# huangnengCSU/NanoSNP

Hardware: AMD Instinct MI355X
Metric: candidate SNP sites/sec (pileup encode + model fwd), 30x windows (higher is better)
Workload: dtype f32; 1 GPU; BASELINE configs[1]: pileup encode + PileupModel fwd, 1M synthetic 30x windows (G2) resident in HBM, batch=4096; batch=4096, windows_resident_per_gpu=1048576, streams=32, precision=fp32, parallelism=site-sharded x1, rooted gather of calls, world_size_observed=1, gather=torch

## Files before the change

nanosnp_amd/csrc/pileup_encode.hip:

```cpp
#include "nsnp_common.hpp"
#include <math.h>

namespace {

enum { CH_A = 0, CH_C, CH_G, CH_T, CH_I, CH_I1, CH_D, CH_D1, CH_STAR,
       CH_a, CH_c, CH_g, CH_t, CH_i, CH_i1, CH_d, CH_d1, CH_POUND, NCH };

constexpr int ENC_BLOCK = 256;
constexpr int MAX_INDEL = 60;

__device__ __forceinline__ int byte_class(int b)
{
    switch (b) {
    case 'A': return 0; case 'C': return 1; case 'G': return 2; case 'T': return 3;
    case 'a': return 4; case 'c': return 5; case 'g': return 6; case 't': return 7;
    case '*': return 8; case '#': return 9;
    case '+': return 11; case '-': return 12; case '^': return 13;
    default: return 10;
    }
}
__device__ __forceinline__ bool is_fwd_char(int b)
{
    return b == 'A' || b == 'C' || b == 'G' || b == 'T' || b == 'N' || b == '*';
}
// ... 73 lines not shown
    Quad t{0, 0, 0, 0};
    for (int64_t i = begin; i < end;) {
        const int b = bases[i];
        const int cls = byte_class(b);
        if (cls < 10) {
            c.k0 += cls == 0; c.k1 += cls == 1; c.k2 += cls == 2; c.k3 += cls == 3; c.k4 += cls == 4;
            c.k5 += cls == 5; c.k6 += cls == 6; c.k7 += cls == 7; c.k8 += cls == 8; c.k9 += cls == 9;
            ++i;
        } else if (cls == 11 || cls == 12) {
            ++i;
            long long adv = 0;
            while (i < end && bases[i] >= '0' && bases[i] <= '9') { adv = adv > 100000000 ? adv : adv * 10 + (bases[i] - '0'); ++i; }
            if (adv <= MAX_INDEL) {
                const int64_t avail = end - i;
                const int len = (int)(adv < avail ? adv : avail);
                t.inc((b == '-' ? 2 : 0) + (len > 0 && is_fwd_char(bases[i]) ? 0 : 1));
            }
            i = adv < end - i ? i + adv : end;
        } else if (cls == 13) i += 2;
        else ++i;
    }
    cnt = c; tot = t;
    mx = rescan_maxima(bases, begin, end);
}

template <typename P>
__device__ __forceinline__ int max_del_exact(P bases, int64_t begin, int64_t end)
{
    int md = 0;
    for (int64_t i = begin; i < end;) {
        const int b = bases[i];
        if (b == '+' || b == '-') {
            ++i;
            long long adv = 0;
            while (i < end && bases[i] >= '0' && bases[i] <= '9') { adv = adv > 100000000 ? adv : adv * 10 + (bases[i] - '0'); ++i; }
            if (b == '-' && adv <= MAX_INDEL && adv > md) md = (int)adv;
            i = adv < end - i ? i + adv : end;
        } else if (b == '^') i += 2;
        else ++i;
    }
    return md;
}

__device__ __forceinline__ bool bed_bit(const uint32_t* __restrict__ bits, int64_t n_bits, int64_t i)
{
    return i >= 0 && i < n_bits && ((bits[i >> 5] >> (i & 31)) & 1u);
}
__device__ __forceinline__ bool bed_any(const uint32_t* __restrict__ bits, int64_t n_bits, int64_t lo, int64_t hi)
{
    if (lo < 0) lo = 0;
    if (hi > n_bits) hi = n_bits;
    if (lo >= hi) return false;
    const int64_t w0 = lo >> 5, w1 = (hi - 1) >> 5;
    for (int64_t w = w0; w <= w1; ++w) {
        uint32_t m = 0xffffffffu;
        if (w == w0) m &= 0xffffffffu << (lo & 31);
        if (w == w1) m &= 0xffffffffu >> (31 - ((hi - 1) & 31));
        if (bits[w] & m) return true;
    }
    return false;
}

constexpr int KEY_SHIFT = 36;
struct BedTable { const uint32_t* words; const int64_t* bed_off; const int64_t* seq_off; int64_t n_contigs; };

__device__ __forceinline__ const uint32_t* bed_table_contig(const BedTable& t, int64_t key, int64_t& n_bits)
{
    const int64_t cid = key >> KEY_SHIFT;
    n_bits = 0;
    if (cid < 0 || cid >= t.n_contigs) return nullptr;
    const int64_t w0 = t.bed_off[cid], cap = (t.bed_off[cid + 1] - w0) * 32, len = t.seq_off[cid + 1] - t.seq_off[cid];
    n_bits = len < cap ? len : cap;
    return t.words + w0;
}
__device__ __forceinline__ int64_t key_pos(int64_t key) { return key & ((1ll << KEY_SHIFT) - 1); }

struct AfThreshold { uint64_t t; int k; int mode; };

static AfThreshold make_af_threshold(double a)
{
    AfThreshold r{0, 0, 0};
    if (a != a) { r.mode = 2; return r; }
    if (a <= 0.0) { r.mode = 1; return r; }
    int e = 0;
    const double m = frexp(a, &e);
    if (!(m > 0.0) || e > 40) { r.mode = 2; return r; }
    const uint64_t M53 = (uint64_t)ldexp(m, 53);
    const bool pow2 = M53 == (1ull << 52);
    r.t = pow2 ? 4 * M53 - 1 : 2 * M53 - 1;
    r.k = (pow2 ? 55 : 54) - e;
    if (r.k >= 88) { r.mode = 1; r.t = 0; r.k = 0; }
    if (r.k < 0) { r.mode = 2; }
    return r;
}

struct AfTable { uint32_t w[128]; };

static AfTable make_af_table(const AfThreshold& af)
{
    AfTable t;
    uint16_t m[256];
    for (int d = 0; d < 256; ++d) {
        m[d] = 0xffff;
        if (af.mode == 1) { m[d] = 1; continue; }
        if (af.mode == 2) continue;
        const unsigned __int128 rhs = (unsigned __int128)af.t * (uint32_t)(d ? d : 1);
        int lo = 1, hi = (d ? d : 1) + 1;
        while (lo < hi) {
            const int c = (lo + hi) >> 1;
            if ((((unsigned __int128)(uint32_t)c) << af.k) >= rhs) hi = c; else lo = c + 1;
        }
        if (lo <= (d ? d : 1)) m[d] = (uint16_t)lo;
    }
    for (int i = 0; i < 128; ++i) t.w[i] = (uint32_t)m[2 * i] | ((uint32_t)m[2 * i + 1] << 16);
    return t;
}

constexpr int ENC_WAVES = ENC_BLOCK / 64;
#ifndef NSNP_ENC_STAGE
#define NSNP_ENC_STAGE 5120
#endif
#ifndef NSNP_ENC_ECAP
#define NSNP_ENC_ECAP 208
#endif
constexpr int STAGE_BYTES = NSNP_ENC_STAGE;
constexpr int ENC_ECAP = NSNP_ENC_ECAP;
#ifndef NSNP_ENC_P3STEP
#define NSNP_ENC_P3STEP 4
#endif
constexpr int P3_STEP = NSNP_ENC_P3STEP;
constexpr int ENC_NBLK = 8;
static_assert(STAGE_BYTES >= 64 * NCH * 4, "the stage buffer doubles as the 64 x 18 output transposition buffer");
static_assert(STAGE_BYTES <= 8192, "staged positions are kept in 13 bits");
static_assert(4 * (ENC_WAVES * (STAGE_BYTES + (ENC_ECAP + P3_STEP) * 8 + 64 * 32) + 4096 + 2 * 512) <= 160 * 1024, "four blocks per CU (LDS)");
constexpr int ENC_ECAP_BED = ENC_ECAP - 32;
static_assert(4 * (ENC_WAVES * (STAGE_BYTES + (ENC_ECAP_BED + P3_STEP) * 8 + 64 * 36) + 4096 + 2 * 512) <= 160 * 1024, "four blocks per CU (LDS)");

struct EncBed { const int64_t* pos; const uint32_t* bits; int64_t n_bits; int32_t* max_del; };
struct EncKeys { const int64_t* key; BedTable tab; int32_t* max_del; };
enum { ENC_PLAIN = 0, ENC_BED = 1, ENC_KEYS = 2 };

__device__ __forceinline__ int wave_scan_incl(int v)
{
    int x = v;
    x += __builtin_amdgcn_update_dpp(0, x, 0x111, 0xf, 0xf, true);
    x += __builtin_amdgcn_update_dpp(0, x, 0x112, 0xf, 0xf, true);
    x += __builtin_amdgcn_update_dpp(0, x, 0x114, 0xf, 0xf, true);
    x += __builtin_amdgcn_update_dpp(0, x, 0x118, 0xf, 0xf, true);
    x += __builtin_amdgcn_update_dpp(0, x, 0x142, 0xa, 0xf, true);
    x += __builtin_amdgcn_update_dpp(0, x, 0x143, 0xc, 0xf, true);
    return x;
}

#ifndef NSNP_ENC_MINW
#define NSNP_ENC_MINW 4
#endif
template <int MODE, typename Bed>
__device__ __forceinline__ void encode_columns_body(
    const uint8_t* __restrict__ bases, const int64_t* __restrict__ col_off, const uint8_t* __restrict__ ref,
    int64_t M, const AfThreshold& af, const AfTable& aft, const AfThreshold& afi, const AfTable& afti, int min_cov, int32_t* __restrict__ counts,
    int32_t* __restrict__ depth_out,
    uint8_t* __restrict__ flags, const Bed& bed)
{
    constexpr bool BED = MODE != ENC_PLAIN;
    constexpr int ECAP = BED ? ENC_ECAP_BED : ENC_ECAP;
    constexpr int NACC = BED ? 9 : 8;
    __shared__ uint32_t af_min[128];
    __shared__ uint32_t afi_min[128];
    __shared__ __attribute__((aligned(16))) uint8_t stage_b[ENC_WAVES][STAGE_BYTES];
    __shared__ uint2 ents[ENC_WAVES][ECAP + P3_STEP];
    __shared__ uint32_t colacc[ENC_WAVES][NACC][64];
    __shared__ uint4 tab[256];
    const int tid = threadIdx.x, lane = tid & 63, wave = tid >> 6;
    {
        const int cls = byte_class(tid);
        uint4 r{0u, 0u, 0u, 0u};
        if (cls < 4) r.x = 1u << (8 * cls);
        else if (cls < 8) r.y = 1u << (8 * (cls - 4));
        else if (cls < 10) r.z = 1u << (8 * (cls - 8));
        else if (cls >= 11) r.w = 1u;
        if (is_fwd_char(tid)) r.z |= 1u << 24;
        tab[tid ^ ((tid >> 2) & 12)] = r;
        if (tid < 128) { af_min[tid] = aft.w[tid]; afi_min[tid] = afti.w[tid]; }
        if (tid < ENC_WAVES * P3_STEP) ents[tid / P3_STEP][tid % P3_STEP] = uint2{0x80000000u, 0u};
    }
    __syncthreads();
    const int64_t wave_col0 = ((int64_t)blockIdx.x * ENC_WAVES + wave) * 64;
    if (wave_col0 >= M) return;
    const int64_t c = wave_col0 + lane;
    const bool live = c < M;
    const int n_live = (int)(M - wave_col0 < 64 ? M - wave_col0 : 64);
    const int64_t* __restrict__ woff = col_off + wave_col0;
    const int64_t wave_end = woff[n_live];
    const int64_t begin64 = woff[lane < n_live ? lane : n_live];
    const int refraw = (ref + wave_col0)[lane < n_live ? lane : n_live - 1];
    const int64_t total = col_off[M];
    const int64_t wave_b0 = __builtin_amdgcn_readfirstlane((int)(begin64 & 0xffffffff)) |
                            ((int64_t)__builtin_amdgcn_readfirstlane((int)(begin64 >> 32)) << 32);
    constexpr int REL_SAT = 1 << 30;
    const int64_t rb64 = begin64 - wave_b0;
    int rbeg = (int)(rb64 < REL_SAT ? rb64 : REL_SAT);
    int rend = __shfl_down(rbeg, 1);
    {
        const int64_t re64 = wave_end - wave_b0;
        if (lane == n_live - 1) rend = (int)(re64 < REL_SAT ? re64 : REL_SAT);
    }
    if (!live) { rbeg = 0; rend = 0; }
    const uint8_t* __restrict__ wbase = bases + wave_b0;

    uint8_t* st = stage_b[wave];
    const uint32_t* st32 = reinterpret_cast<const uint32_t*>(st);
    uint2* ent = ents[wave] + P3_STEP;
    uint32_t (*const cacc)[64] = colacc[wave];
    int32_t cnt[10];
#pragma unroll
    for (int k = 0; k < 10; ++k) cnt[k] = 0;
    Quad tot{0, 0, 0, 0};
    Quad mx{0, 0, 0, 0};
    bool slow = false;
    int mdel = 0;

    for (int first = 0; first < n_live;) {
        const int b0 = __builtin_amdgcn_readlane(rbeg, first);
        const int mis = (int)((uintptr_t)(wbase + b0) & 15);
        const uint8_t* __restrict__ src = wbase + (b0 - mis);
        const bool fits = live && lane >= first && b0 < REL_SAT && rend <= (STAGE_BYTES - 16 - mis) + b0 && rend >= b0;
        const unsigned long long fm = __ballot(fits) >> first;
        int n_fit = (~fm) ? __builtin_ctzll(~fm) : 64;
        if (n_fit > n_live - first) n_fit = n_live - first;
        if (n_fit == 0) {
            if (lane == first) slow = true;
            first += 1;
            continue;
        }
        const int last = first + n_fit;
        const int span = __builtin_amdgcn_readlane(rend, last - 1) - b0 + mis;
        {
            const bool inside = (uintptr_t)src >= (uintptr_t)bases && (uintptr_t)src + (((uintptr_t)span + 15) & ~(uintptr_t)15) <= (uintptr_t)(bases + total);
            if (inside) {
                constexpr int NP = (STAGE_BYTES + 1023) / 1024;
                const int o_last = ((span - 1) >> 4) << 4;
                uint4 pc[NP];
#pragma unroll
                for (int i = 0; i < NP; ++i) { const int o = (lane + 64 * i) * 16; pc[i] = *reinterpret_cast<const uint4*>(src + (o < span ? o : o_last)); }
#pragma unroll
                for (int i = 0; i < NP; ++i) { const int o = (lane + 64 * i) * 16; if (o < span) *reinterpret_cast<uint4*>(st + o) = pc[i]; }
            } else {
                for (int o = lane * 16; o < span; o += 64 * 16) {
                    uint32_t wv[4] = {0u, 0u, 0u, 0u};
                    for (int k = 0; k < 16; ++k) {
                        const uint8_t* q = src + o + k;
                        if (q >= bases && q < bases + total) wv[k >> 2] |= (uint32_t)(*q) << (8 * (k & 3));
                    }
                    *reinterpret_cast<uint4*>(st + o) = uint4{wv[0], wv[1], wv[2], wv[3]};
                }
            }
        }
#pragma unroll
        for (int k = 0; k < NACC; ++k) cacc[k][lane] = 0u;
        __builtin_amdgcn_fence(__ATOMIC_RELEASE, "wavefront");
        __builtin_amdgcn_wave_barrier();

        {
            const bool act = lane >= first && lane < last;
            const int lbeg = act ? rbeg - b0 + mis : mis, lend = act ? rend - b0 + mis : mis;
            const int wb = lbeg & ~3;
            const int tr = act ? ((lend - 1 - wb) >> 2) : -1;
            bool bad = tr >= 8 * ENC_NBLK || lend - lbeg > 253;
            const int trp = bad ? -1 : tr;
            const uint32_t hm = (1u << (8 * (lbeg & 3))) - 1u;
            const int rem = lend - (wb + 4 * tr);
            const uint32_t tm = rem >= 4 ? 0u : 0xffffffffu << (8 * (rem & 3));
            const uint32_t* cw = st32 + (wb >> 2);
            uint32_t ax = 0, ay = 0, az = 0;
            uint32_t sm[ENC_NBLK];
#pragma unroll
            for (int b = 0; b < ENC_NBLK; ++b) sm[b] = 0u;
#pragma unroll
            for (int b = 0; b < ENC_NBLK; ++b) {
                if (__ballot(trp >= 8 * b) == 0ull) break;
                uint32_t smb = 0u;
#pragma nounroll
                for (int r = 0; r < 8; r += 2) {
#pragma unroll
                    for (int h = 0; h < 2; ++h) {
                        const int R = 8 * b + r + h;
                        uint32_t w = cw[R];
                        w |= (R == 0) ? hm : 0u;
                        w |= R < trp ? 0u : (R == trp ? tm : 0xffffffffu);
                        w ^= (w >> 2) & 0x0c0c0c0cu;
                        const uint4 r0 = tab[w & 0xffu], r1 = tab[(w >> 8) & 0xffu], r2 = tab[(w >> 16) & 0xffu], r3 = tab[w >> 24];
                        ax += r0.x + r1.x; ax += r2.x + r3.x;
                        ay += r0.y + r1.y; ay += r2.y + r3.y;
                        az += r0.z + r1.z; az += r2.z + r3.z;
                        const uint32_t f4 = (((r3.w << 1) | r2.w) << 2) | ((r1.w << 1) | r0.w);
                        smb |= f4 << (4 * (r + h));
                    }
                    if (__ballot(trp > 8 * b + r + 1) == 0ull) break;
                }
                sm[b] = smb;
            }
            int n_op = 0;
#pragma unroll
            for (int b = 0; b < ENC_NBLK; ++b) n_op += __builtin_popcount(sm[b]);
            if (n_op > ECAP) { bad = true; n_op = 0; }
            const int incl = wave_scan_incl(n_op);
            const int excl = incl - n_op;
            const int total_ops = __builtin_amdgcn_readlane(incl, 63);
            for (int sfirst = first; total_ops > 0 && sfirst < last;) {
                const int sbase = __shfl(excl, sfirst);
                const bool sfit = act && lane >= sfirst && incl - sbase <= ECAP;
                const unsigned long long sfm = __ballot(sfit) >> sfirst;
                int n_seg = (~sfm) ? __builtin_ctzll(~sfm) : 64;
                if (n_seg > last - sfirst) n_seg = last - sfirst;
                const int slast = sfirst + n_seg;
                const int T = __shfl(incl, slast - 1) - sbase;
                const bool sact = lane >= sfirst && lane < slast;
                {
                    int j = excl - sbase;
                    const uint32_t tag = (uint32_t)wb | ((uint32_t)lane << 16);
#pragma unroll
                    for (int b = 0; b < ENC_NBLK; ++b) {
                        uint32_t cur = (sact && n_op > 0) ? sm[b] : 0u;
                        while (__ballot(cur != 0u) != 0ull) {
                            if (cur != 0u) {
                                ent[j] = uint2{tag + (uint32_t)(32 * b + __builtin_ctz(cur)), (uint32_t)lend};
                                cur &= cur - 1u; ++j;
                            }
                        }
                    }
                }
                __builtin_amdgcn_fence(__ATOMIC_RELEASE, "wavefront");
                __builtin_amdgcn_wave_barrier();
                int n_cnt = 0;
                for (int r0i = 0; r0i < T; r0i += 64) {
                    const int j = r0i + lane;
                    const bool valid = j < T;
                    uint2 e0 = ent[valid ? j : 0];
                    if (!valid) e0 = uint2{0u, 0u};
                    const int p = e0.x & 0xffff, owner = (int)(e0.x >> 16), lend_o = (int)e0.y;
                    const int b = st[p];
                    const int w0 = (p + 1) >> 2;
                    const uint32_t a0 = st32[w0], a1 = st32[w0 + 1], a2 = st32[w0 + 2];
                    const int sh = (p + 1) & 3;
                    const uint32_t wlo = __builtin_amdgcn_alignbyte(a1, a0, sh), whi = __builtin_amdgcn_alignbyte(a2, a1, sh);
                    const int avail1 = lend_o - (p + 1);
                    const bool caret = b == '^';
                    const uint32_t d0 = (wlo & 0xffu) - '0', d1 = ((wlo >> 8) & 0xffu) - '0', d2 = ((wlo >> 16) & 0xffu) - '0', d3 = (wlo >> 24) - '0';
                    const bool k0 = !caret && avail1 > 0 && d0 < 10u, k1 = k0 && avail1 > 1 && d1 < 10u, k2 = k1 && avail1 > 2 && d2 < 10u;
                    const bool mybad = k2 && avail1 > 3 && d3 < 10u;
                    const int L = k2 ? 3 : (k1 ? 2 : (k0 ? 1 : 0));
                    const int adv = caret ? 1 : (k2 ? (int)(d0 * 100 + d1 * 10 + d2) : (k1 ? (int)(d0 * 10 + d1) : (k0 ? (int)d0 : 0)));
                    const int q = p + 1 + L;
                    const int avail = lend_o - q;
                    const int nskip = adv < avail ? adv : (avail > 0 ? avail : 0);
                    const uint32_t al = __builtin_amdgcn_alignbyte(whi, wlo, L);
                    const uint32_t keep = nskip >= 4 ? 0xffffffffu : ((1u << (8 * (nskip & 3))) - 1u);
                    const uint32_t alm = al | ~keep;
                    const uint32_t alp = alm ^ ((alm >> 2) & 0x0c0c0c0cu);
                    const uint4 r0 = tab[alp & 0xffu], r1 = tab[(alp >> 8) & 0xffu], r2 = tab[(alp >> 16) & 0xffu], r3 = tab[alp >> 24];
                    const bool counted = valid && !caret && adv <= MAX_INDEL;
                    uint32_t nx = r0.x + r1.x, ny = r0.y + r1.y, nz = r0.z + r1.z;
                    nx += r2.x + r3.x; ny += r2.y + r3.y; nz += r2.z + r3.z;
                    uint32_t inner = (r0.w | r1.w) | (r2.w | r3.w);
                    if (valid) {
                        for (int k = q + 4; k < q + nskip; ++k) {
                            const uint32_t bk = st[k];
                            const uint4 rr = tab[bk ^ ((bk >> 2) & 12u)];
                            nx += rr.x; ny += rr.y; nz += rr.z; inner |= rr.w;
                        }
                        atomicAdd(&cacc[0][owner], nx); atomicAdd(&cacc[1][owner], ny);
                        if (nz & 0xffffffu) atomicAdd(&cacc[2][owner], nz & 0xffffffu);
                        if (mybad || inner || (counted && adv > nskip)) atomicOr(&cacc[2][owner], 0x80000000u);
                        if (BED) { if (counted && b == '-') atomicMax(&cacc[NACC - 1][owner], (uint32_t)adv); }
                    }
                    const unsigned long long cm = __ballot(counted);
                    const uint32_t fwd = (r0.z >> 24) & 1u;
                    if (counted)
                        ent[n_cnt + (int)__builtin_amdgcn_mbcnt_hi((uint32_t)(cm >> 32), __builtin_amdgcn_mbcnt_lo((uint32_t)cm, 0u))] =
                            uint2{(uint32_t)q | ((uint32_t)nskip << 13) | ((uint32_t)(b == '-') << 19) | (fwd << 20) | ((uint32_t)owner << 25), al & keep};
                    n_cnt += __builtin_popcountll(cm);
                }
                __builtin_amdgcn_fence(__ATOMIC_RELEASE, "wavefront");
                __builtin_amdgcn_wave_barrier();
                for (int r0i = 0; r0i < n_cnt; r0i += 64) {
                    const int j = r0i + lane;
                    bool go = j < n_cnt;
                    const uint2* f = ent + (go ? j : 0);
                    const uint2 me = *f;
                    const int le = (me.x >> 13) & 63, qe = me.x & 0x1fff;
                    int same = 1;
                    while (__ballot(go) != 0ull) {
                        if (go) {
                            f -= P3_STEP;
                            uint2 o[P3_STEP];
#pragma unroll
                            for (int u = 0; u < P3_STEP; ++u) o[u] = f[P3_STEP - 1 - u];
                            uint32_t hit = 0u;
#pragma unroll
                            for (int u = 0; u < P3_STEP; ++u) {
                                const uint32_t t = o[u].x ^ me.x;
                                go = go && t < (1u << 25);
                                hit |= (uint32_t)(go && t < (1u << 13) && o[u].y == me.y) << u;
                            }
                            same += __builtin_popcount(hit);
                            if (le > 4) {
                                for (; hit; hit &= hit - 1u) {
                                    const int qf = f[P3_STEP - 1 - __builtin_ctz(hit)].x & 0x1fff;
                                    for (int k = 4; k < le; ++k) if (st[qe + k] != st[qf + k]) { --same; break; }
                                }
                            }
                        }
                    }
                    if (j < n_cnt) {
                        const int kind = (int)((me.x >> 19) & 1u) * 2 + (int)(((me.x >> 20) & 1u) ^ 1u);
                        const int col = (int)(me.x >> 25);
                        atomicAdd(&cacc[3][col], 1u << (8 * kind));
                        atomicMax(&cacc[4 + kind][col], (uint32_t)same);
                    }
                }
                __builtin_amdgcn_fence(__ATOMIC_RELEASE, "wavefront");
                __builtin_amdgcn_wave_barrier();
                sfirst = slast;
            }
            __builtin_amdgcn_fence(__ATOMIC_ACQUIRE, "wavefront");
            {
                const uint4 a0 = uint4{cacc[0][lane], cacc[1][lane], cacc[2][lane], cacc[3][lane]};
                const uint4 a1 = uint4{cacc[4][lane], cacc[5][lane], cacc[6][lane], cacc[7][lane]};
                ax -= a0.x; ay -= a0.y; az -= a0.z;
                if (act) {
                    cnt[0] = ax & 0xff; cnt[1] = (ax >> 8) & 0xff; cnt[2] = (ax >> 16) & 0xff; cnt[3] = ax >> 24;
                    cnt[4] = ay & 0xff; cnt[5] = (ay >> 8) & 0xff; cnt[6] = (ay >> 16) & 0xff; cnt[7] = ay >> 24;
                    cnt[8] = az & 0xff; cnt[9] = (az >> 8) & 0xff;
                    tot = Quad{(int)(a0.w & 0xff), (int)((a0.w >> 8) & 0xff), (int)((a0.w >> 16) & 0xff), (int)(a0.w >> 24)};
                    mx = Quad{(int)a1.x, (int)a1.y, (int)a1.z, (int)a1.w};
                    if (BED) mdel = (int)cacc[NACC - 1][lane];
                }
                bad = bad || (act && (a0.z >> 31));
            }
            if (bad) {
                Counts10 c2; Quad t2, m2;
                scan_column_exact((const uint8_t*)st, (int64_t)lbeg, (int64_t)lend, c2, t2, m2);
                cnt[0] = c2.k0; cnt[1] = c2.k1; cnt[2] = c2.k2; cnt[3] = c2.k3; cnt[4] = c2.k4;
                cnt[5] = c2.k5; cnt[6] = c2.k6; cnt[7] = c2.k7; cnt[8] = c2.k8; cnt[9] = c2.k9;
                tot = t2; mx = m2;
                if (BED) mdel = max_del_exact((const uint8_t*)st, (int64_t)lbeg, (int64_t)lend);
            }
        }
        __builtin_amdgcn_wave_barrier();
        first = last;
    }
    if (slow) {
        Counts10 c2; Quad t2, m2;
        scan_column_exact(bases, begin64, lane == n_live - 1 ? wave_end : woff[lane + 1], c2, t2, m2);
        cnt[0] = c2.k0; cnt[1] = c2.k1; cnt[2] = c2.k2; cnt[3] = c2.k3; cnt[4] = c2.k4;
        cnt[5] = c2.k5; cnt[6] = c2.k6; cnt[7] = c2.k7; cnt[8] = c2.k8; cnt[9] = c2.k9;
        tot = t2; mx = m2;
        if (BED) mdel = max_del_exact(bases, begin64, lane == n_live - 1 ? wave_end : woff[lane + 1]);
    }

    int32_t t[NCH];
    t[CH_A] = cnt[0]; t[CH_C] = cnt[1]; t[CH_G] = cnt[2]; t[CH_T] = cnt[3];
    t[CH_a] = cnt[4]; t[CH_c] = cnt[5]; t[CH_g] = cnt[6]; t[CH_t] = cnt[7];
    t[CH_STAR] = cnt[8]; t[CH_POUND] = cnt[9];
    t[CH_I] = tot.v0; t[CH_i] = tot.v1; t[CH_D] = tot.v2; t[CH_d] = tot.v3;
    t[CH_I1] = mx.v0; t[CH_i1] = mx.v1; t[CH_D1] = mx.v2; t[CH_d1] = mx.v3;
    const int up = cnt[0] + cnt[1] + cnt[2] + cnt[3];
    const int lo = cnt[4] + cnt[5] + cnt[6] + cnt[7];
    const int depth = up + lo + cnt[8] + cnt[9];
    const int rb = nt4(refraw);
    const int chr_idx = rb < 4 ? rb : 0;
    const int lc[6] = {cnt[0] + cnt[4], cnt[1] + cnt[5], tot.v2 + tot.v3, cnt[2] + cnt[6], tot.v0 + tot.v1, cnt[3] + cnt[7]};
    const int lk[6] = {0, 1, 5, 2, 4, 3};
    int top = -1, topc = 0;
#pragma unroll
    for (int k = 0; k < 6; ++k) if (lc[k] > topc) { topc = lc[k]; top = lk[k]; }
    bool pass_snp = false, pass_indel = false;
    if (__ballot(depth > 255) == 0ull) {
        const int thr = (int)((af_min[depth >> 1] >> (16 * (depth & 1))) & 0xffffu);
        const int thri = (int)((afi_min[depth >> 1] >> (16 * (depth & 1))) & 0xffffu);
#pragma unroll
        for (int k = 0; k < 6; ++k) {
            const bool cand = lc[k] > 0 && lk[k] != chr_idx;
            if (lk[k] >= 4) pass_indel = pass_indel || (cand && lc[k] >= thri); else pass_snp = pass_snp || (cand && lc[k] >= thr);
        }
    } else {
        const uint32_t den = (uint32_t)(depth ? depth : 1);
        const unsigned __int128 rhs = (unsigned __int128)af.t * den, rhsi = (unsigned __int128)afi.t * den;
#pragma unroll
        for (int k = 0; k < 6; ++k) {
            if (lc[k] <= 0 || lk[k] == chr_idx) continue;
            if (lk[k] >= 4) pass_indel = pass_indel || (afi.mode == 0 ? (((unsigned __int128)(uint32_t)lc[k] << afi.k) >= rhsi) : afi.mode == 1);
            else pass_snp = pass_snp || (af.mode == 0 ? (((unsigned __int128)(uint32_t)lc[k] << af.k) >= rhs) : af.mode == 1);
        }
    }
    const bool pass_af = (top >= 0 && top != chr_idx) || pass_snp || pass_indel;
    const int up_ch[4] = {CH_A, CH_C, CH_G, CH_T}, lo_ch[4] = {CH_a, CH_c, CH_g, CH_t};
#pragma unroll
    for (int k = 0; k < 4; ++k) if (k == chr_idx) { t[up_ch[k]] = -up; t[lo_ch[k]] = -lo; }

    __builtin_amdgcn_wave_barrier();
    int32_t* out_stage = reinterpret_cast<int32_t*>(st);
#pragma unroll
    for (int k = 0; k < NCH; k += 2) *reinterpret_cast<int2*>(out_stage + lane * NCH + k) = int2{t[k], t[k + 1]};
    __builtin_amdgcn_fence(__ATOMIC_RELEASE, "wavefront");
    __builtin_amdgcn_wave_barrier();
    const int n_valid = n_live * NCH;
    int32_t* __restrict__ dst = counts + wave_col0 * NCH;
    if ((reinterpret_cast<uintptr_t>(dst) & 15) == 0) {
        const int n16 = n_valid >> 2;
        for (int k = lane; k < n16; k += 64) reinterpret_cast<int4*>(dst)[k] = reinterpret_cast<const int4*>(out_stage)[k];
        for (int k = (n16 << 2) + lane; k < n_valid; k += 64) dst[k] = out_stage[k];
    } else {
        for (int k = lane; k < n_valid; k += 64) dst[k] = out_stage[k];
    }
    if (live) {
        (depth_out + wave_col0)[lane] = depth;
        uint8_t f = 0;
        if (pass_af) f |= NSNP_FLAG_PASS_AF;
        if (pass_snp) f |= NSNP_FLAG_PASS_SNP;
        if (pass_indel) f |= NSNP_FLAG_PASS_INDEL;
        bool cand = rb < 4 && pass_af && depth >= min_cov;
        if (BED) {
            if (bed.max_del) (bed.max_del + wave_col0)[lane] = mdel;
            if constexpr (MODE == ENC_KEYS) {
                if (cand && bed.tab.bed_off) {
                    const int64_t k = (bed.key + wave_col0)[lane];
                    int64_t nb;
                    const uint32_t* w = bed_table_contig(bed.tab, k, nb);
                    const int64_t p = key_pos(k);
                    cand = bed_any(w, nb, p - 1, p + mdel + 1);
                }
            } else {
                if (cand && bed.bits) { const int64_t p = (bed.pos + wave_col0)[lane]; cand = bed_any(bed.bits, bed.n_bits, p - 1, p + mdel + 1); }
            }
        }
        if (cand) f |= NSNP_FLAG_CANDIDATE;
        (flags + wave_col0)[lane] = f;
    }
}

__global__ __launch_bounds__(ENC_BLOCK, NSNP_ENC_MINW) void k_encode_columns(
    const uint8_t* __restrict__ bases, const int64_t* __restrict__ col_off, const uint8_t* __restrict__ ref,
    int64_t M, AfThreshold af, const AfTable aft, AfThreshold afi, const AfTable afti, int min_cov, int32_t* __restrict__ counts,
    int32_t* __restrict__ depth_out,
    uint8_t* __restrict__ flags)
{
    encode_columns_body<ENC_PLAIN>(bases, col_off, ref, M, af, aft, afi, afti, min_cov, counts, depth_out, flags, EncBed{nullptr, nullptr, 0, nullptr});
}

__global__ __launch_bounds__(ENC_BLOCK, NSNP_ENC_MINW) void k_encode_columns_bed(
    const uint8_t* __restrict__ bases, const int64_t* __restrict__ col_off, const uint8_t* __restrict__ ref,
    int64_t M, AfThreshold af, const AfTable aft, AfThreshold afi, const AfTable afti, int min_cov, int32_t* __restrict__ counts,
    int32_t* __restrict__ depth_out,
    uint8_t* __restrict__ flags, const EncBed bed)
{
    encode_columns_body<ENC_BED>(bases, col_off, ref, M, af, aft, afi, afti, min_cov, counts, depth_out, flags, bed);
}

__global__ __launch_bounds__(ENC_BLOCK, NSNP_ENC_MINW) void k_encode_columns_keys(
    const uint8_t* __restrict__ bases, const int64_t* __restrict__ col_off, const uint8_t* __restrict__ ref,
    int64_t M, AfThreshold af, const AfTable aft, AfThreshold afi, const AfTable afti, int min_cov, int32_t* __restrict__ counts,
    int32_t* __restrict__ depth_out,
    uint8_t* __restrict__ flags, const EncKeys bed)
{
    encode_columns_body<ENC_KEYS>(bases, col_off, ref, M, af, aft, afi, afti, min_cov, counts, depth_out, flags, bed);
}


__device__ __forceinline__ bool site_ok(const int64_t* pos, const uint8_t* flags, int64_t M, int64_t c)
{
    if (!(flags[c] & NSNP_FLAG_CANDIDATE)) return false;
    if (c < PCENTER || c + PCENTER >= M) return false;
    if (!(pos[c + PCENTER] - pos[c] == PCENTER && pos[c] - pos[c - PCENTER] == PCENTER)) return false;
    int64_t p[2 * PCENTER + 1];
#pragma unroll
    for (int k = 0; k <= 2 * PCENTER; ++k) p[k] = pos[c - PCENTER + k];
    bool bad = false;
#pragma unroll
    for (int k = 0; k < 2 * PCENTER; ++k) bad |= p[k + 1] - p[k] != 1;
    return !bad;
}

constexpr int SEL_BLOCK = 256, SEL_PER_THREAD = 8, SEL_TILE = SEL_BLOCK * SEL_PER_THREAD;

__global__ __launch_bounds__(SEL_BLOCK) void k_select_count(const int64_t* pos, const uint8_t* flags, int64_t M,
                                                             int64_t* block_cnt)
{
    __shared__ int wsum[SEL_BLOCK / 64];
    const int64_t base = (int64_t)blockIdx.x * SEL_TILE + threadIdx.x;
    int n = 0;
#pragma unroll
    for (int k = 0; k < SEL_PER_THREAD; ++k) { const int64_t c = base + (int64_t)k * SEL_BLOCK; if (c < M && site_ok(pos, flags, M, c)) ++n; }
    for (int o = 32; o > 0; o >>= 1) n += __shfl_down(n, o);
    if ((threadIdx.x & 63) == 0) wsum[threadIdx.x >> 6] = n;
    __syncthreads();
    if (threadIdx.x == 0) { int s = 0; for (int w = 0; w < SEL_BLOCK / 64; ++w) s += wsum[w]; block_cnt[blockIdx.x] = s; }
}

__global__ __launch_bounds__(1024) void k_select_scan(int64_t* block_cnt, int64_t n_blocks, int64_t* total)
{
    __shared__ int64_t part[1024];
    const int tid = threadIdx.x;
    const int64_t per = NSNP_CDIV(n_blocks, 1024);
    const int64_t b0 = tid * per, b1 = (b0 + per < n_blocks) ? b0 + per : n_blocks;
    int64_t s = 0;
    for (int64_t b = b0; b < b1; ++b) s += block_cnt[b];
    part[tid] = s;
    __syncthreads();
    for (int o = 1; o < 1024; o <<= 1) {
        int64_t v = tid >= o ? part[tid - o] : 0;
        __syncthreads();
        part[tid] += v;
        __syncthreads();
    }
    int64_t run = tid ? part[tid - 1] : 0;
    for (int64_t b = b0; b < b1; ++b) { const int64_t v = block_cnt[b]; block_cnt[b] = run; run += v; }
    if (tid == 1023) *total = part[1023];
}

__global__ __launch_bounds__(SEL_BLOCK) void k_select_scatter(const int64_t* pos, const uint8_t* flags, int64_t M,
                                                               const int64_t* block_off, int64_t* center_idx, int64_t cap)
{
    __shared__ int wcnt[SEL_PER_THREAD][SEL_BLOCK / 64];
    const int tid = threadIdx.x, lane = tid & 63, wave = tid >> 6;
    const int64_t base = (int64_t)blockIdx.x * SEL_TILE + tid;
    unsigned okm = 0; int before[SEL_PER_THREAD];
#pragma unroll
    for (int k = 0; k < SEL_PER_THREAD; ++k) {
        const int64_t c = base + (int64_t)k * SEL_BLOCK;
        const bool ok = c < M && site_ok(pos, flags, M, c);
        const unsigned long long bal = __ballot(ok);
        before[k] = __popcll(bal & ((1ull << lane) - 1ull));
        if (lane == 0) wcnt[k][wave] = __popcll(bal);
        okm |= (unsigned)ok << k;
    }
    __syncthreads();
    int run = 0;
#pragma unroll
    for (int k = 0; k < SEL_PER_THREAD; ++k) {
#pragma unroll
        for (int w = 0; w < SEL_BLOCK / 64; ++w) {
            if (w == wave && ((okm >> k) & 1u)) {
                const int64_t o = block_off[blockIdx.x] + run + before[k];
                if (o < cap) center_idx[o] = base + (int64_t)k * SEL_BLOCK;
            }
            run += wcnt[k][w];
        }
    }
}

__global__ void k_gather_windows(const int32_t* __restrict__ counts, const int64_t* __restrict__ center_idx, int64_t N,
                                 int32_t* __restrict__ x)
{
    constexpr int W = PW * PC;
    const int64_t total = N * W;
    for (int64_t e = (int64_t)blockIdx.x * blockDim.x + threadIdx.x; e < total; e += (int64_t)gridDim.x * blockDim.x) {
        const int64_t n = e / W; const int r = (int)(e - n * W);
        x[e] = counts[(center_idx[n] - PCENTER) * PC + r];
    }
}

}

static int encode_columns_launch(nsnp_ctx* ctx, const uint8_t* bases, const int64_t* col_off,
                                 const uint8_t* ref, int64_t M, double snp_min_af, double indel_min_af, int min_coverage,
                                 int32_t* counts, int32_t* depth, uint8_t* flags, const EncBed* bed, void* stream, const EncKeys* keys = nullptr)
{
    if (!ctx || M < 0 || (M > 0 && (!bases || !col_off || !ref || !counts || !depth || !flags))) return NSNP_EINVAL;
    if (M == 0) return NSNP_OK;
    const unsigned grid = (unsigned)NSNP_CDIV(M, ENC_BLOCK);
    ScopedKernelTimer tm(ctx, NSNP_K_ENCODE, (hipStream_t)stream);
    static_assert(sizeof(AfTable) == sizeof(ctx->af_table_words), "AfTable is 128 words");
    uint64_t af_bits; memcpy(&af_bits, &snp_min_af, 8);
    if (!ctx->af_cached || ctx->af_bits != af_bits) {
        const AfThreshold a0 = make_af_threshold(snp_min_af);
        const AfTable t0 = make_af_table(a0);
        ctx->af_t = a0.t; ctx->af_k = a0.k; ctx->af_mode = a0.mode;
        memcpy(ctx->af_table_words, t0.w, sizeof(t0.w));
        ctx->af_bits = af_bits; ctx->af_cached = true;
    }
    uint64_t af2_bits; memcpy(&af2_bits, &indel_min_af, 8);
    if (!ctx->af2_cached || ctx->af2_bits != af2_bits) {
        const AfThreshold a0 = make_af_threshold(indel_min_af);
        const AfTable t0 = make_af_table(a0);
        ctx->af2_t = a0.t; ctx->af2_k = a0.k; ctx->af2_mode = a0.mode;
        memcpy(ctx->af2_table_words, t0.w, sizeof(t0.w));
        ctx->af2_bits = af2_bits; ctx->af2_cached = true;
    }
    AfThreshold af{ctx->af_t, ctx->af_k, ctx->af_mode}, afi{ctx->af2_t, ctx->af2_k, ctx->af2_mode};
    AfTable aft, afti; memcpy(aft.w, ctx->af_table_words, sizeof(aft.w)); memcpy(afti.w, ctx->af2_table_words, sizeof(afti.w));
    if (keys)
// ... 363 lines not shown
```

Before: 21.47 million sites/s.

## Restructure pileup encode kernel with per-chunk finish, DPP shifts and bit tricks

Moves the per-column finalisation (AF test, flag and count output) inside the chunk loop so each fitting chunk writes its outputs directly, and handles slow columns immediately instead of after the loop. It also loads the byte-class table from a constexpr device image, uses a DPP row shift instead of a shuffle, and zeroes the accumulators with 16-byte stores. Indel-digit parsing becomes SWAR plus udot4, and the flag bits are packed with v_lshl_or and a bit reverse. The goal is fewer instructions and registers in the encode kernel, at the cost of more code paths and more complex output stores that could diverge for partial waves.

```diff
diff --git a/nanosnp_amd/csrc/pileup_encode.hip b/nanosnp_amd/csrc/pileup_encode.hip
--- a/nanosnp_amd/csrc/pileup_encode.hip
+++ b/nanosnp_amd/csrc/pileup_encode.hip
@@ -249,6 +249,25 @@
     return x;
 }
 
+struct TabRow { uint32_t x, y, z, w; };
+struct TabImage { TabRow r[256]; };
+constexpr TabImage make_tab_image()
+{
+    TabImage t{};
+    for (int b = 0; b < 256; ++b) {
+        TabRow r{0u, 0u, 0u, 0u};
+        const char up[4] = {'A', 'C', 'G', 'T'}, lo[4] = {'a', 'c', 'g', 't'};
+        for (int k = 0; k < 4; ++k) { if (b == up[k]) r.x = 1u << (8 * k); if (b == lo[k]) r.y = 1u << (8 * k); }
+        if (b == '*') r.z = 1u;
+        if (b == '#') r.z = 1u << 8;
+        if (b == '+' || b == '-' || b == '^') r.w = 1u;
+        if (b == 'A' || b == 'C' || b == 'G' || b == 'T' || b == 'N' || b == '*') r.z |= 1u << 24;
+        t.r[b ^ ((b >> 2) & 12)] = r;
+    }
+    return t;
+}
+__device__ __attribute__((aligned(16))) const TabImage k_enc_tab = make_tab_image();
+
 #ifndef NSNP_ENC_MINW
 #define NSNP_ENC_MINW 4
 #endif
@@ -266,27 +285,20 @@
     __shared__ uint32_t afi_min[128];
     __shared__ __attribute__((aligned(16))) uint8_t stage_b[ENC_WAVES][STAGE_BYTES];
     __shared__ uint2 ents[ENC_WAVES][ECAP + P3_STEP];
-    __shared__ uint32_t colacc[ENC_WAVES][NACC][64];
+    __shared__ __attribute__((aligned(16))) uint32_t colacc[ENC_WAVES][NACC][64];
     __shared__ uint4 tab[256];
-    const int tid = threadIdx.x, lane = tid & 63, wave = tid >> 6;
+    const int tid = threadIdx.x, lane = tid & 63, wave = __builtin_amdgcn_readfirstlane(tid >> 6);
     {
-        const int cls = byte_class(tid);
-        uint4 r{0u, 0u, 0u, 0u};
-        if (cls < 4) r.x = 1u << (8 * cls);
-        else if (cls < 8) r.y = 1u << (8 * (cls - 4));
-        else if (cls < 10) r.z = 1u << (8 * (cls - 8));
-        else if (cls >= 11) r.w = 1u;
-        if (is_fwd_char(tid)) r.z |= 1u << 24;
-        tab[tid ^ ((tid >> 2) & 12)] = r;
+        static_assert(ENC_BLOCK == 256, "one table row per thread");
+        tab[tid] = reinterpret_cast<const uint4*>(k_enc_tab.r)[tid];
         if (tid < 128) { af_min[tid] = aft.w[tid]; afi_min[tid] = afti.w[tid]; }
         if (tid < ENC_WAVES * P3_STEP) ents[tid / P3_STEP][tid % P3_STEP] = uint2{0x80000000u, 0u};
     }
     __syncthreads();
     const int64_t wave_col0 = ((int64_t)blockIdx.x * ENC_WAVES + wave) * 64;
     if (wave_col0 >= M) return;
-    const int64_t c = wave_col0 + lane;
-    const bool live = c < M;
     const int n_live = (int)(M - wave_col0 < 64 ? M - wave_col0 : 64);
+    const bool live = lane < n_live;
     const int64_t* __restrict__ woff = col_off + wave_col0;
     const int64_t wave_end = woff[n_live];
     const int64_t begin64 = woff[lane < n_live ? lane : n_live];
@@ -297,7 +309,7 @@
     constexpr int REL_SAT = 1 << 30;
     const int64_t rb64 = begin64 - wave_b0;
     int rbeg = (int)(rb64 < REL_SAT ? rb64 : REL_SAT);
-    int rend = __shfl_down(rbeg, 1);
+    int rend = __builtin_amdgcn_update_dpp(rbeg, rbeg, 0x130, 0xf, 0xf, false);
     {
         const int64_t re64 = wave_end - wave_b0;
         if (lane == n_live - 1) rend = (int)(re64 < REL_SAT ? re64 : REL_SAT);
@@ -309,13 +321,72 @@
     const uint32_t* st32 = reinterpret_cast<const uint32_t*>(st);
     uint2* ent = ents[wave] + P3_STEP;
     uint32_t (*const cacc)[64] = colacc[wave];
-    int32_t cnt[10];
-#pragma unroll
-    for (int k = 0; k < 10; ++k) cnt[k] = 0;
-    Quad tot{0, 0, 0, 0};
-    Quad mx{0, 0, 0, 0};
-    bool slow = false;
-    int mdel = 0;
+    auto finish = [&](const int32_t (&cnt)[10], const Quad& tot, const Quad& mx, const int mdel, const bool mine, int32_t (&t)[NCH])
+                  __attribute__((always_inline)) {
+        t[CH_A] = cnt[0]; t[CH_C] = cnt[1]; t[CH_G] = cnt[2]; t[CH_T] = cnt[3];
+        t[CH_a] = cnt[4]; t[CH_c] = cnt[5]; t[CH_g] = cnt[6]; t[CH_t] = cnt[7];
+        t[CH_STAR] = cnt[8]; t[CH_POUND] = cnt[9];
+        t[CH_I] = tot.v0; t[CH_i] = tot.v1; t[CH_D] = tot.v2; t[CH_d] = tot.v3;
+        t[CH_I1] = mx.v0; t[CH_i1] = mx.v1; t[CH_D1] = mx.v2; t[CH_d1] = mx.v3;
+        const int up = cnt[0] + cnt[1] + cnt[2] + cnt[3];
+        const int lo = cnt[4] + cnt[5] + cnt[6] + cnt[7];
+        const int depth = up + lo + cnt[8] + cnt[9];
+        const int rb = nt4(refraw);
+        const int chr_idx = rb < 4 ? rb : 0;
+        const int lc[6] = {cnt[0] + cnt[4], cnt[1] + cnt[5], tot.v2 + tot.v3, cnt[2] + cnt[6], tot.v0 + tot.v1, cnt[3] + cnt[7]};
+        const int lk[6] = {0, 1, 5, 2, 4, 3};
+        int top = -1, topc = 0;
+    #pragma unroll
+        for (int k = 0; k < 6; ++k) if (lc[k] > topc) { topc = lc[k]; top = lk[k]; }
+        bool pass_snp = false, pass_indel = false;
+        if (__ballot(depth > 255) == 0ull) {
+            const int thr = (int)((af_min[depth >> 1] >> (16 * (depth & 1))) & 0xffffu);
+            const int thri = (int)((afi_min[depth >> 1] >> (16 * (depth & 1))) & 0xffffu);
+    #pragma unroll
+            for (int k = 0; k < 6; ++k) {
+                const bool cand = lk[k] != chr_idx;
+                if (lk[k] >= 4) pass_indel = pass_indel || (cand && lc[k] >= thri); else pass_snp = pass_snp || (cand && lc[k] >= thr);
+            }
+        } else {
+            const uint32_t den = (uint32_t)(depth ? depth : 1);
+            const unsigned __int128 rhs = (unsigned __int128)af.t * den, rhsi = (unsigned __int128)afi.t * den;
+    #pragma unroll
+            for (int k = 0; k < 6; ++k) {
+                if (lc[k] <= 0 || lk[k] == chr_idx) continue;
+                if (lk[k] >= 4) pass_indel = pass_indel || (afi.mode == 0 ? (((unsigned __int128)(uint32_t)lc[k] << afi.k) >= rhsi) : afi.mode == 1);
+                else pass_snp = pass_snp || (af.mode == 0 ? (((unsigned __int128)(uint32_t)lc[k] << af.k) >= rhs) : af.mode == 1);
+            }
+        }
+        const bool pass_af = (top >= 0 && top != chr_idx) || pass_snp || pass_indel;
+        const int up_ch[4] = {CH_A, CH_C, CH_G, CH_T}, lo_ch[4] = {CH_a, CH_c, CH_g, CH_t};
+    #pragma unroll
+        for (int k = 0; k < 4; ++k) if (k == chr_idx) { t[up_ch[k]] = -up; t[lo_ch[k]] = -lo; }
+
+        if (mine) {
+            (depth_out + wave_col0)[lane] = depth;
+            uint8_t f = 0;
+            if (pass_af) f |= NSNP_FLAG_PASS_AF;
+            if (pass_snp) f |= NSNP_FLAG_PASS_SNP;
+            if (pass_indel) f |= NSNP_FLAG_PASS_INDEL;
+            bool cand = rb < 4 && pass_af && depth >= min_cov;
+            if (BED) {
+                if (bed.max_del) (bed.max_del + wave_col0)[lane] = mdel;
+                if constexpr (MODE == ENC_KEYS) {
+                    if (cand && bed.tab.bed_off) {
+                        const int64_t k = (bed.key + wave_col0)[lane];
+                        int64_t nb;
+                        const uint32_t* w = bed_table_contig(bed.tab, k, nb);
+                        const int64_t p = key_pos(k);
+                        cand = bed_any(w, nb, p - 1, p + mdel + 1);
+                    }
+                } else {
+                    if (cand && bed.bits) { const int64_t p = (bed.pos + wave_col0)[lane]; cand = bed_any(bed.bits, bed.n_bits, p - 1, p + mdel + 1); }
+                }
+            }
+            if (cand) f |= NSNP_FLAG_CANDIDATE;
+            (flags + wave_col0)[lane] = f;
+        }
+    };
 
     for (int first = 0; first < n_live;) {
         const int b0 = __builtin_amdgcn_readlane(rbeg, first);
@@ -326,7 +397,18 @@
         int n_fit = (~fm) ? __builtin_ctzll(~fm) : 64;
         if (n_fit > n_live - first) n_fit = n_live - first;
         if (n_fit == 0) {
-            if (lane == first) slow = true;
+            if (lane == first) {
+                const int64_t end64 = lane == n_live - 1 ? wave_end : woff[lane + 1];
+                Counts10 c2; Quad t2, m2;
+                scan_column_exact(bases, begin64, end64, c2, t2, m2);
+                const int32_t cnt[10] = {c2.k0, c2.k1, c2.k2, c2.k3, c2.k4, c2.k5, c2.k6, c2.k7, c2.k8, c2.k9};
+                const int mdel = BED ? max_del_exact(bases, begin64, end64) : 0;
+                int32_t t[NCH];
+                finish(cnt, t2, m2, mdel, true, t);
+                int32_t* __restrict__ row = counts + (wave_col0 + lane) * NCH;
+#pragma unroll
+                for (int k = 0; k < NCH; ++k) row[k] = t[k];
+            }
             first += 1;
             continue;
         }
@@ -353,8 +435,12 @@
                 }
             }
         }
-#pragma unroll
-        for (int k = 0; k < NACC; ++k) cacc[k][lane] = 0u;
+        {
+            uint4* z4 = reinterpret_cast<uint4*>(&cacc[0][0]);
+            static_assert(NACC * 64 * 4 % 16 == 0 && sizeof(colacc[0]) % 16 == 0, "whole 16-byte pieces, every wave's part aligned");
+#pragma unroll
+            for (int i = 0; i < NACC * 16; i += 64) if (i + 64 <= NACC * 16 || lane < NACC * 16 - i) z4[i + lane] = uint4{0u, 0u, 0u, 0u};
+        }
         __builtin_amdgcn_fence(__ATOMIC_RELEASE, "wavefront");
         __builtin_amdgcn_wave_barrier();
 
@@ -373,12 +459,15 @@
             uint32_t sm[ENC_NBLK];
 #pragma unroll
             for (int b = 0; b < ENC_NBLK; ++b) sm[b] = 0u;
+            int nblk = 0;
 #pragma unroll
             for (int b = 0; b < ENC_NBLK; ++b) {
                 if (__ballot(trp >= 8 * b) == 0ull) break;
+                nblk = b + 1;
                 uint32_t smb = 0u;
+                int r = 0;
 #pragma nounroll
-                for (int r = 0; r < 8; r += 2) {
+                do {
 #pragma unroll
                     for (int h = 0; h < 2; ++h) {
                         const int R = 8 * b + r + h;
@@ -390,16 +479,18 @@
                         ax += r0.x + r1.x; ax += r2.x + r3.x;
                         ay += r0.y + r1.y; ay += r2.y + r3.y;
                         az += r0.z + r1.z; az += r2.z + r3.z;
-                        const uint32_t f4 = (((r3.w << 1) | r2.w) << 2) | ((r1.w << 1) | r0.w);
-                        smb |= f4 << (4 * (r + h));
+                        asm("v_lshl_or_b32 %0, %0, 1, %1" : "+v"(smb) : "v"(r0.w));
+                        asm("v_lshl_or_b32 %0, %0, 1, %1" : "+v"(smb) : "v"(r1.w));
+                        asm("v_lshl_or_b32 %0, %0, 1, %1" : "+v"(smb) : "v"(r2.w));
+                        asm("v_lshl_or_b32 %0, %0, 1, %1" : "+v"(smb) : "v"(r3.w));
                     }
-                    if (__ballot(trp > 8 * b + r + 1) == 0ull) break;
-                }
-                sm[b] = smb;
+                    r += 2;
+                } while (r < 8 && __ballot(trp >= 8 * b + r) != 0ull);
+                sm[b] = __builtin_bitreverse32(smb << (4 * (8 - r)));
             }
             int n_op = 0;
 #pragma unroll
-            for (int b = 0; b < ENC_NBLK; ++b) n_op += __builtin_popcount(sm[b]);
+            for (int b = 0; b < ENC_NBLK; ++b) { if (b >= nblk) break; n_op += __builtin_popcount(sm[b]); }
             if (n_op > ECAP) { bad = true; n_op = 0; }
             const int incl = wave_scan_incl(n_op);
             const int excl = incl - n_op;
@@ -414,15 +505,17 @@
                 const int T = __shfl(incl, slast - 1) - sbase;
                 const bool sact = lane >= sfirst && lane < slast;
                 {
-                    int j = excl - sbase;
+                    uint2* ep = ent + (excl - sbase);
                     const uint32_t tag = (uint32_t)wb | ((uint32_t)lane << 16);
+                    const bool mine = sact && n_op > 0;
 #pragma unroll
                     for (int b = 0; b < ENC_NBLK; ++b) {
-                        uint32_t cur = (sact && n_op > 0) ? sm[b] : 0u;
+                        if (b >= nblk) break;
+                        uint32_t cur = mine ? sm[b] : 0u;
                         while (__ballot(cur != 0u) != 0ull) {
                             if (cur != 0u) {
-                                ent[j] = uint2{tag + (uint32_t)(32 * b + __builtin_ctz(cur)), (uint32_t)lend};
-                                cur &= cur - 1u; ++j;
+                                *ep++ = uint2{tag + (uint32_t)(32 * b + __builtin_ctz(cur)), (uint32_t)lend};
+                                cur &= cur - 1u;
                             }
                         }
                     }
@@ -434,7 +527,7 @@
                     const int j = r0i + lane;
                     const bool valid = j < T;
                     uint2 e0 = ent[valid ? j : 0];
-                    if (!valid) e0 = uint2{0u, 0u};
+                    if (!valid) e0 = uint2{0u, 1u};
                     const int p = e0.x & 0xffff, owner = (int)(e0.x >> 16), lend_o = (int)e0.y;
                     const int b = st[p];
                     const int w0 = (p + 1) >> 2;
@@ -443,11 +536,13 @@
                     const uint32_t wlo = __builtin_amdgcn_alignbyte(a1, a0, sh), whi = __builtin_amdgcn_alignbyte(a2, a1, sh);
                     const int avail1 = lend_o - (p + 1);
                     const bool caret = b == '^';
-                    const uint32_t d0 = (wlo & 0xffu) - '0', d1 = ((wlo >> 8) & 0xffu) - '0', d2 = ((wlo >> 16) & 0xffu) - '0', d3 = (wlo >> 24) - '0';
-                    const bool k0 = !caret && avail1 > 0 && d0 < 10u, k1 = k0 && avail1 > 1 && d1 < 10u, k2 = k1 && avail1 > 2 && d2 < 10u;
-                    const bool mybad = k2 && avail1 > 3 && d3 < 10u;
-                    const int L = k2 ? 3 : (k1 ? 2 : (k0 ? 1 : 0));
-                    const int adv = caret ? 1 : (k2 ? (int)(d0 * 100 + d1 * 10 + d2) : (k1 ? (int)(d0 * 10 + d1) : (k0 ? (int)d0 : 0)));
+                    const uint32_t dg = wlo ^ 0x30303030u;
+                    const uint32_t nd = (((dg & 0x7f7f7f7fu) + 0x76767676u) | dg) & 0x80808080u;
+                    const uint32_t run = nd ? (uint32_t)__builtin_ctz(nd) >> 3 : 4u;
+                    const uint32_t Lraw = run < (uint32_t)avail1 ? run : (uint32_t)avail1;
+                    const bool mybad = !caret && Lraw >= 4u;
+                    const int L = caret ? 0 : (int)(Lraw < 3u ? Lraw : 3u);
+                    const int adv = caret ? 1 : (int)__builtin_amdgcn_udot4(dg << (8 * (3 - L)), 0x00010a64u, 0u, false);
                     const int q = p + 1 + L;
                     const int avail = lend_o - q;
                     const int nskip = adv < avail ? adv : (avail > 0 ? avail : 0);
@@ -521,18 +616,19 @@
                 sfirst = slast;
             }
             __builtin_amdgcn_fence(__ATOMIC_ACQUIRE, "wavefront");
+            int32_t cnt[10];
+            Quad tot, mx;
+            int mdel = 0;
             {
                 const uint4 a0 = uint4{cacc[0][lane], cacc[1][lane], cacc[2][lane], cacc[3][lane]};
                 const uint4 a1 = uint4{cacc[4][lane], cacc[5][lane], cacc[6][lane], cacc[7][lane]};
                 ax -= a0.x; ay -= a0.y; az -= a0.z;
-                if (act) {
-                    cnt[0] = ax & 0xff; cnt[1] = (ax >> 8) & 0xff; cnt[2] = (ax >> 16) & 0xff; cnt[3] = ax >> 24;
-                    cnt[4] = ay & 0xff; cnt[5] = (ay >> 8) & 0xff; cnt[6] = (ay >> 16) & 0xff; cnt[7] = ay >> 24;
-                    cnt[8] = az & 0xff; cnt[9] = (az >> 8) & 0xff;
-                    tot = Quad{(int)(a0.w & 0xff), (int)((a0.w >> 8) & 0xff), (int)((a0.w >> 16) & 0xff), (int)(a0.w >> 24)};
-                    mx = Quad{(int)a1.x, (int)a1.y, (int)a1.z, (int)a1.w};
-                    if (BED) mdel = (int)cacc[NACC - 1][lane];
-                }
+                cnt[0] = ax & 0xff; cnt[1] = (ax >> 8) & 0xff; cnt[2] = (ax >> 16) & 0xff; cnt[3] = ax >> 24;
+                cnt[4] = ay & 0xff; cnt[5] = (ay >> 8) & 0xff; cnt[6] = (ay >> 16) & 0xff; cnt[7] = ay >> 24;
+                cnt[8] = az & 0xff; cnt[9] = (az >> 8) & 0xff;
+                tot = Quad{(int)(a0.w & 0xff), (int)((a0.w >> 8) & 0xff), (int)((a0.w >> 16) & 0xff), (int)(a0.w >> 24)};
+                mx = Quad{(int)a1.x, (int)a1.y, (int)a1.z, (int)a1.w};
+                if (BED) mdel = (int)cacc[NACC - 1][lane];
                 bad = bad || (act && (a0.z >> 31));
             }
             if (bad) {
@@ -543,98 +639,44 @@
                 tot = t2; mx = m2;
                 if (BED) mdel = max_del_exact((const uint8_t*)st, (int64_t)lbeg, (int64_t)lend);
             }
+            int32_t t[NCH];
+            finish(cnt, tot, mx, mdel, act, t);
+            __builtin_amdgcn_wave_barrier();
+            int32_t* out_stage = reinterpret_cast<int32_t*>(st);
+#pragma unroll
+            for (int k = 0; k < NCH; k += 2) *reinterpret_cast<int2*>(out_stage + lane * NCH + k) = int2{t[k], t[k + 1]};
+            __builtin_amdgcn_fence(__ATOMIC_RELEASE, "wavefront");
+            __builtin_amdgcn_wave_barrier();
+            int32_t* __restrict__ dst = counts + wave_col0 * NCH;
+            const bool al16 = (reinterpret_cast<uintptr_t>(dst) & 15) == 0;
+            if (first == 0 && last == 64 && al16) {
+                const int4* s4 = reinterpret_cast<const int4*>(out_stage) + lane;
+                int4* d4 = reinterpret_cast<int4*>(dst) + lane;
+                constexpr int ROWS = 64 * NCH / 4 / 64;
+                static_assert(64 * NCH / 4 == ROWS * 64 + 32, "4 1/2 rows");
+                int4 v[ROWS + 1];
+#pragma unroll
+                for (int i = 0; i < ROWS; ++i) v[i] = s4[64 * i];
+                if (lane < 32) v[ROWS] = s4[64 * ROWS];
+#pragma unroll
+                for (int i = 0; i < ROWS; ++i) d4[64 * i] = v[i];
+                if (lane < 32) d4[64 * ROWS] = v[ROWS];
+            } else {
+                int ln = lane;
+                asm volatile("" : "+v"(ln));
+                if (first == 0 && al16) {
+                    const int n_valid = last * NCH, n16 = n_valid >> 2;
+                    for (int k = ln; k < n16; k += 64) reinterpret_cast<int4*>(dst)[k] = reinterpret_cast<const int4*>(out_stage)[k];
+                    for (int k = (n16 << 2) + ln; k < n_valid; k += 64) dst[k] = out_stage[k];
+                } else {
+                    for (int k = first * NCH + ln; k < last * NCH; k += 64) dst[k] = out_stage[k];
+                }
+            }
         }
         __builtin_amdgcn_wave_barrier();
         first = last;
     }
-    if (slow) {
-        Counts10 c2; Quad t2, m2;
-        scan_column_exact(bases, begin64, lane == n_live - 1 ? wave_end : woff[lane + 1], c2, t2, m2);
-        cnt[0] = c2.k0; cnt[1] = c2.k1; cnt[2] = c2.k2; cnt[3] = c2.k3; cnt[4] = c2.k4;
-        cnt[5] = c2.k5; cnt[6] = c2.k6; cnt[7] = c2.k7; cnt[8] = c2.k8; cnt[9] = c2.k9;
-        tot = t2; mx = m2;
-        if (BED) mdel = max_del_exact(bases, begin64, lane == n_live - 1 ? wave_end : woff[lane + 1]);
-    }
-
-    int32_t t[NCH];
-    t[CH_A] = cnt[0]; t[CH_C] = cnt[1]; t[CH_G] = cnt[2]; t[CH_T] = cnt[3];
-    t[CH_a] = cnt[4]; t[CH_c] = cnt[5]; t[CH_g] = cnt[6]; t[CH_t] = cnt[7];
-    t[CH_STAR] = cnt[8]; t[CH_POUND] = cnt[9];
-    t[CH_I] = tot.v0; t[CH_i] = tot.v1; t[CH_D] = tot.v2; t[CH_d] = tot.v3;
-    t[CH_I1] = mx.v0; t[CH_i1] = mx.v1; t[CH_D1] = mx.v2; t[CH_d1] = mx.v3;
-    const int up = cnt[0] + cnt[1] + cnt[2] + cnt[3];
-    const int lo = cnt[4] + cnt[5] + cnt[6] + cnt[7];
-    const int depth = up + lo + cnt[8] + cnt[9];
-    const int rb = nt4(refraw);
-    const int chr_idx = rb < 4 ? rb : 0;
-    const int lc[6] = {cnt[0] + cnt[4], cnt[1] + cnt[5], tot.v2 + tot.v3, cnt[2] + cnt[6], tot.v0 + tot.v1, cnt[3] + cnt[7]};
-    const int lk[6] = {0, 1, 5, 2, 4, 3};
-    int top = -1, topc = 0;
-#pragma unroll
-    for (int k = 0; k < 6; ++k) if (lc[k] > topc) { topc = lc[k]; top = lk[k]; }
-    bool pass_snp = false, pass_indel = false;
-    if (__ballot(depth > 255) == 0ull) {
-        const int thr = (int)((af_min[depth >> 1] >> (16 * (depth & 1))) & 0xffffu);
-        const int thri = (int)((afi_min[depth >> 1] >> (16 * (depth & 1))) & 0xffffu);
-#pragma unroll
-        for (int k = 0; k < 6; ++k) {
-            const bool cand = lc[k] > 0 && lk[k] != chr_idx;
-            if (lk[k] >= 4) pass_indel = pass_indel || (cand && lc[k] >= thri); else pass_snp = pass_snp || (cand && lc[k] >= thr);
-        }
-    } else {
-        const uint32_t den = (uint32_t)(depth ? depth : 1);
-        const unsigned __int128 rhs = (unsigned __int128)af.t * den, rhsi = (unsigned __int128)afi.t * den;
-#pragma unroll
-        for (int k = 0; k < 6; ++k) {
-            if (lc[k] <= 0 || lk[k] == chr_idx) continue;
-            if (lk[k] >= 4) pass_indel = pass_indel || (afi.mode == 0 ? (((unsigned __int128)(uint32_t)lc[k] << afi.k) >= rhsi) : afi.mode == 1);
-            else pass_snp = pass_snp || (af.mode == 0 ? (((unsigned __int128)(uint32_t)lc[k] << af.k) >= rhs) : af.mode == 1);
-        }
-    }
-    const bool pass_af = (top >= 0 && top != chr_idx) || pass_snp || pass_indel;
-    const int up_ch[4] = {CH_A, CH_C, CH_G, CH_T}, lo_ch[4] = {CH_a, CH_c, CH_g, CH_t};
-#pragma unroll
-    for (int k = 0; k < 4; ++k) if (k == chr_idx) { t[up_ch[k]] = -up; t[lo_ch[k]] = -lo; }
-
-    __builtin_amdgcn_wave_barrier();
-    int32_t* out_stage = reinterpret_cast<int32_t*>(st);
-#pragma unroll
-    for (int k = 0; k < NCH; k += 2) *reinterpret_cast<int2*>(out_stage + lane * NCH + k) = int2{t[k], t[k + 1]};
-    __builtin_amdgcn_fence(__ATOMIC_RELEASE, "wavefront");
-    __builtin_amdgcn_wave_barrier();
-    const int n_valid = n_live * NCH;
-    int32_t* __restrict__ dst = counts + wave_col0 * NCH;
-    if ((reinterpret_cast<uintptr_t>(dst) & 15) == 0) {
-        const int n16 = n_valid >> 2;
-        for (int k = lane; k < n16; k += 64) reinterpret_cast<int4*>(dst)[k] = reinterpret_cast<const int4*>(out_stage)[k];
-        for (int k = (n16 << 2) + lane; k < n_valid; k += 64) dst[k] = out_stage[k];
-    } else {
-        for (int k = lane; k < n_valid; k += 64) dst[k] = out_stage[k];
-    }
-    if (live) {
-        (depth_out + wave_col0)[lane] = depth;
-        uint8_t f = 0;
-        if (pass_af) f |= NSNP_FLAG_PASS_AF;
-        if (pass_snp) f |= NSNP_FLAG_PASS_SNP;
-        if (pass_indel) f |= NSNP_FLAG_PASS_INDEL;
-        bool cand = rb < 4 && pass_af && depth >= min_cov;
-        if (BED) {
-            if (bed.max_del) (bed.max_del + wave_col0)[lane] = mdel;
-            if constexpr (MODE == ENC_KEYS) {
-                if (cand && bed.tab.bed_off) {
-                    const int64_t k = (bed.key + wave_col0)[lane];
-                    int64_t nb;
-                    const uint32_t* w = bed_table_contig(bed.tab, k, nb);
-                    const int64_t p = key_pos(k);
-                    cand = bed_any(w, nb, p - 1, p + mdel + 1);
-                }
-            } else {
-                if (cand && bed.bits) { const int64_t p = (bed.pos + wave_col0)[lane]; cand = bed_any(bed.bits, bed.n_bits, p - 1, p + mdel + 1); }
-            }
-        }
-        if (cand) f |= NSNP_FLAG_CANDIDATE;
-        (flags + wave_col0)[lane] = f;
-    }
+
 }
 
 __global__ __launch_bounds__(ENC_BLOCK, NSNP_ENC_MINW) void k_encode_columns(
```

Measured after the change: 21.51 million sites/s, median of 6. No clear change (+0.2%).
